# Zokrates/ZoKrates

Hardware: NVIDIA H100
Metric: groth16_constraints_per_sec (higher is better)
Workload: dtype u256-montgomery

## Files before the change

### zokrates_b200/csrc/engine.cuh

```cuda
#pragma once
#include <map>
#include <memory>
#include <vector>
#include <chrono>
#include <cmath>
#include <future>
#include "fp64.cuh"
#include "msm.cuh"
#include "msm_affine.cuh"
#include "ntt.cuh"
#include "ntt_tile.cuh"
#include "solvers.cuh"
#include "rt.cuh"
#include "engine_base.cuh"

#ifndef ZKB_G2_MINB
#define ZKB_G2_MINB 2
#endif

namespace zkb {

struct k_fr_convert; struct k_spmv; struct k_ntt_dif; struct k_ntt_dit; struct k_ntt_scale; struct k_ntt_brev;
struct k_ntt_table; struct k_qap_pointwise; struct k_msm_digits; struct k_msm_scatter; struct k_msm_accum1;
struct k_msm_accum2; struct k_msm_bitsum; struct k_pk_convert; struct k_final_a; struct k_final_b;
struct k_final_c; struct k_final_d; struct k_point_out; struct k_field_op; struct k_setup_scalars; struct k_fixed_base;
struct k_to_affine; struct k_copy; struct k_msm_view; struct k_solver_level; struct k_ba_halve; struct k_ba_round; struct k_msm_table; struct k_ntt_dif_tile; struct k_ntt_dit_tile; struct k_witness_level;

struct StageTimer {
#if !defined(ZKB_EMU)
  struct Ev { const char* name; cudaEvent_t a, b; };
  std::vector<Ev> evs;
  std::vector<size_t> open;
  Stream st;
  explicit StageTimer(Stream s) : st(s) {}
  void begin(const char* name) {
    Ev e{name, nullptr, nullptr};
    ZKB_CUDA(cudaEventCreate(&e.a));
    ZKB_CUDA(cudaEventCreate(&e.b));
    ZKB_CUDA(cudaEventRecord(e.a, st.s));
    open.push_back(evs.size());
    evs.push_back(e);
  }
  void end() {
    size_t i = open.back();
    open.pop_back();
    ZKB_CUDA(cudaEventRecord(evs[i].b, st.s));
  }
  size_t begin_on(Stream s, const char* name) {
    Ev e{name, nullptr, nullptr};
    ZKB_CUDA(cudaEventCreate(&e.a));
    ZKB_CUDA(cudaEventCreate(&e.b));
    ZKB_CUDA(cudaEventRecord(e.a, s.s));
    evs.push_back(e);
    return evs.size() - 1;
  }
  void end_on(Stream s, size_t i) { ZKB_CUDA(cudaEventRecord(evs[i].b, s.s)); }
  void collect(std::vector<std::pair<const char*, double>>& out) {
    out.clear();
    for (auto& e : evs) {
      ZKB_CUDA(cudaEventSynchronize(e.b));
      float ms = 0;
      ZKB_CUDA(cudaEventElapsedTime(&ms, e.a, e.b));
      out.push_back({e.name, (double)ms});
      cudaEventDestroy(e.a);
      cudaEventDestroy(e.b);
    }
    evs.clear();
  }
  ~StageTimer() { for (auto& e : evs) { cudaEventDestroy(e.a); cudaEventDestroy(e.b); } }
#else
  explicit StageTimer(Stream) {}
  void begin(const char*) {}
  void end() {}
  size_t begin_on(Stream, const char*) { return 0; }
  void end_on(Stream, size_t) {}
  void collect(std::vector<std::pair<const char*, double>>& out) { out.clear(); }
#endif
};

#if !defined(ZKB_EMU)
static __global__ void zkb_scan_kernel(const uint32_t* counts, uint32_t* offsets, uint32_t n) {
  __shared__ uint32_t sums[1024];
  const uint32_t tid = threadIdx.x;
  const uint32_t per = (n + 1023u) / 1024u;
  const uint32_t lo = tid * per < n ? tid * per : n;
  const uint32_t hi = lo + per < n ? lo + per : n;
  uint32_t s = 0;
  for (uint32_t i = lo; i < hi; i++) s += counts[i];
  sums[tid] = s;
  __syncthreads();
  for (uint32_t off = 1; off < 1024; off <<= 1) {
    uint32_t v = tid >= off ? sums[tid - off] : 0;
    __syncthreads();
    sums[tid] += v;
    __syncthreads();
  }
  uint32_t base = tid ? sums[tid - 1] : 0;
  for (uint32_t i = lo; i < hi; i++) {
    offsets[i] = base;
    base += counts[i];
  }
  if (tid == 1023) offsets[n] = sums[1023];
}
#endif
#if !defined(ZKB_EMU)
static constexpr int SCAN_BLOCK = 256, SCAN_PER = 8, SCAN_TILE = SCAN_BLOCK * SCAN_PER;
static __global__ void zkb_scan_tile_sums(const uint32_t* in, uint32_t* tile_sums, uint32_t n) {
  __shared__ uint32_t red[SCAN_BLOCK / 32];
  const uint32_t base = blockIdx.x * SCAN_TILE + threadIdx.x * SCAN_PER;
  uint32_t s = 0;
#pragma unroll
  for (int k = 0; k < SCAN_PER; k++) s += (base + k < n) ? in[base + k] : 0;
  for (int off = 16; off; off >>= 1) s += __shfl_down_sync(0xffffffffu, s, off);
  if ((threadIdx.x & 31) == 0) red[threadIdx.x >> 5] = s;
  __syncthreads();
  if (threadIdx.x == 0) {
    uint32_t t = 0;
    for (int k = 0; k < SCAN_BLOCK / 32; k++) t += red[k];
    tile_sums[blockIdx.x] = t;
  }
}
static __global__ void zkb_scan_tile_apply(const uint32_t* in, const uint32_t* tile_offsets, uint32_t* out, uint32_t n,
                                           uint32_t ntiles) {
  __shared__ uint32_t wsum[SCAN_BLOCK / 32];
  const uint32_t base = blockIdx.x * SCAN_TILE + threadIdx.x * SCAN_PER;
  uint32_t v[SCAN_PER], s = 0;
#pragma unroll
  for (int k = 0; k < SCAN_PER; k++) { v[k] = (base + k < n) ? in[base + k] : 0; s += v[k]; }
  uint32_t incl = s;
  const uint32_t lane = threadIdx.x & 31, warp = threadIdx.x >> 5;
  for (int off = 1; off < 32; off <<= 1) { uint32_t y = __shfl_up_sync(0xffffffffu, incl, off); if (lane >= (uint32_t)off) incl += y; }
  if (lane == 31) wsum[warp] = incl;
  __syncthreads();
  uint32_t wbase = 0;
  for (uint32_t k = 0; k < warp; k++) wbase += wsum[k];
  uint32_t run = tile_offsets[blockIdx.x] + wbase + incl - s;
#pragma unroll
  for (int k = 0; k < SCAN_PER; k++) { if (base + k < n) out[base + k] = run; run += v[k]; }
  if (blockIdx.x == ntiles - 1 && threadIdx.x == SCAN_BLOCK - 1) out[n] = tile_offsets[ntiles];
}
#endif
inline void exclusive_scan(Stream st, const uint32_t* counts, uint32_t* offsets, uint32_t n, uint32_t* tile_tmp = nullptr) {
#if !defined(ZKB_EMU)
  if (tile_tmp && n > 4096) {
    const uint32_t ntiles = (n + SCAN_TILE - 1) / SCAN_TILE;
    launch_counter() += 3;
    zkb_scan_tile_sums<<<ntiles, SCAN_BLOCK, 0, st.s>>>(counts, tile_tmp, n);
    zkb_scan_kernel<<<1, 1024, 0, st.s>>>(tile_tmp, tile_tmp + ntiles + 1, ntiles);
    zkb_scan_tile_apply<<<ntiles, SCAN_BLOCK, 0, st.s>>>(counts, tile_tmp + ntiles + 1, offsets, n, ntiles);
    ZKB_CUDA(cudaGetLastError());
    return;
  }
  launch_counter()++;
  zkb_scan_kernel<<<1, 1024, 0, st.s>>>(counts, offsets, n);
  ZKB_CUDA(cudaGetLastError());
#else
  (void)tile_tmp;
  uint32_t base = 0;
  for (uint32_t i = 0; i < n; i++) { offsets[i] = base; base += counts[i]; }
  offsets[n] = base;
#endif
}

static constexpr int VIEW_BLOCK = 256, VIEW_ITERS = 8, VIEW_TILE = VIEW_BLOCK * VIEW_ITERS, VIEW_GROUPS = VIEW_TILE / 32;
#if !defined(ZKB_EMU)
static __global__ void __launch_bounds__(VIEW_BLOCK) zkb_view_count(MsmShape sh, const uint8_t* skip, const uint32_t* sorted0,
                                                                    const uint32_t* offsets0, uint32_t NB, uint32_t* tile_cnt,
                                                                    uint32_t ntiles) {
  __shared__ uint32_t cnt[2];
  if (threadIdx.x < 2) cnt[threadIdx.x] = 0;
  __syncthreads();
// ... 733 lines not shown
    pl.sh.W = (C::FR_BITS + 1 + c - 1) / c;
    pl.sh.B = 1u << (c - 1);
    pl.nbuckets = msm_nbuckets(pl.sh);
    uint64_t total = n * pl.sh.W;
    if (total * nviews >= (1ull << 32)) throw Error(ZKB_E_ARG, "msm too large");
    uint64_t target = (uint64_t)opts.chunk_target;
    uint64_t T = (total + target - 1) / target;
    if (T < 8) T = 8;
    if (T > 64) T = 64;
    T = (T + 1) & ~1ull;
    pl.T1 = (uint32_t)T;
    pl.T2 = 8;
    pl.nt1 = (uint32_t)((total + pl.T1 - 1) / pl.T1);
    const uint32_t NB = pl.nbuckets;
    if (nviews > 3) throw Error(ZKB_E_INTERNAL, "at most two filtered views");
    pl.digits.ensure(total); pl.ranks.ensure(total); pl.sorted.ensure(total * nviews);
    pl.counts.ensure(NB); pl.offsets.ensure((size_t)(NB + 1) * nviews);
    dev_zero(st_, pl.counts.p, (size_t)NB * 4);
    MsmShape sh = pl.sh;
    const uint32_t* sc = (const uint32_t*)scalars;
    uint32_t* dg = pl.digits.p; uint32_t* rk = pl.ranks.p; uint32_t* cn = pl.counts.p; uint32_t* of = pl.offsets.p;
    uint32_t* so = pl.sorted.p;
    launch<k_msm_digits>(st_, n, ZKB_LAMBDA(size_t t) { msm_digits_body(sh, sc, dg, rk, cn, (uint32_t)t); });
    const uint32_t ntiles = (uint32_t)((total + VIEW_TILE - 1) / VIEW_TILE);
    pl.scan_tmp.ensure(2 * ((size_t)(NB > ntiles ? NB : ntiles) / 2048 + 4));
    exclusive_scan(st_, cn, of, NB, pl.scan_tmp.p);
    launch<k_msm_scatter>(st_, total, ZKB_LAMBDA(size_t t) { msm_scatter_body(sh, dg, rk, of, so, t); });
    if (nviews > 1) build_views(pl, skip, total, ntiles);
  }

  void build_views(MsmPlan& pl, const uint8_t* skip, uint64_t total, uint32_t ntiles) {
    const uint32_t NB = pl.nbuckets, nv = pl.nviews - 1;
    const MsmShape sh = pl.sh;
    const uint32_t* of0 = pl.offsets.p;
    const uint32_t* so0 = pl.sorted.p;
    uint32_t* sov = pl.sorted.p + total;
#if !defined(ZKB_EMU)
    const uint32_t ngroups = (uint32_t)((total + 31) / 32);
    pl.view_tile_cnt.ensure((size_t)2 * ntiles); pl.view_tile_off.ensure((size_t)2 * (ntiles + 1));
    pl.view_pre32.ensure((size_t)2 * ngroups); pl.view_mask32.ensure((size_t)2 * ngroups);
    launch_counter() += 2;
    zkb_view_count<<<ntiles, VIEW_BLOCK, 0, st_.s>>>(sh, skip, so0, of0, NB, pl.view_tile_cnt.p, ntiles);
    ZKB_CUDA(cudaGetLastError());
    for (uint32_t v = 0; v < nv; v++)
      exclusive_scan(st_, pl.view_tile_cnt.p + (size_t)v * ntiles, pl.view_tile_off.p + (size_t)v * (ntiles + 1), ntiles, pl.scan_tmp.p);
    zkb_view_apply<<<ntiles, VIEW_BLOCK, 0, st_.s>>>(sh, skip, so0, of0, NB, nv, pl.view_tile_off.p, ntiles, sov, (size_t)total,
                                                     pl.view_pre32.p, pl.view_mask32.p, ngroups);
    ZKB_CUDA(cudaGetLastError());
    for (uint32_t v = 0; v < nv; v++) {
      const uint32_t* pre = pl.view_pre32.p + (size_t)v * ngroups; const uint32_t* msk = pl.view_mask32.p + (size_t)v * ngroups;
      const uint32_t* tot = pl.view_tile_off.p + (size_t)v * (ntiles + 1) + ntiles;
      uint32_t* ofv = pl.offsets.p + (size_t)(v + 1) * (NB + 1);
      launch<k_msm_view>(st_, (size_t)NB + 1, ZKB_LAMBDA(size_t t) { msm_view_offsets_body(NB, of0, pre, msk, tot, ofv, (uint32_t)t); });
    }
#else
    (void)ntiles;
    const uint32_t M = of0[NB];
    for (uint32_t v = 0; v < nv; v++) {
      uint32_t* ofv = pl.offsets.p + (size_t)(v + 1) * (NB + 1);
      uint32_t* out = sov + (size_t)v * total;
      uint32_t kept = 0, b = 0;
      for (uint32_t p = 0; p <= M; p++) {
        while (b <= NB && of0[b] == p) ofv[b++] = kept;
        if (p < M && msm_view_keep(sh, skip, so0[p], v + 1)) out[kept++] = so0[p];
      }
    }
#endif
  }

  MsmWs ws_misc_;
  Stream wm_stream_, plan_stream_;
  bool has_wm_stream_ = false, has_plan_stream_ = false;
  struct StreamScope {
    Stream& ref; Stream saved;
    StreamScope(Stream& r, Stream s) : ref(r), saved(r) { ref = s; }
    ~StreamScope() { ref = saved; }
  };
  Stream tail_stream(MsmWs& ws) {
    if (!ws.has_stream) { ws.tail = stream_create_high_priority(); ws.has_stream = true; }
    return ws.tail;
  }
  ~Engine() override {
    if (prepared_.fut.valid()) prepared_.fut.wait();
    for (auto& sl : slots_) { if (sl.fm.valid()) sl.fm.wait(); sl.destroy(); }
    ws_misc_.destroy();
    if (has_wm_stream_) stream_destroy(wm_stream_);
    if (has_plan_stream_) stream_destroy(plan_stream_);
  }

  DevBuf<uint8_t> ba_pts_[2];
  DevBuf<uint32_t> ba_off_[2], ba_cnt_, ba_scan_tmp_;

  template <class F>
  void msm_accumulate(const MsmPlan& pl, const Affine<F>* pts, MsmWs& ws, StageTimer* tm, const char* accum_name, uint32_t view) {
    typedef XYZZ<F> X;
    if (pl.sh.n == 0) return;
    const uint32_t NB = pl.nbuckets;
    ws.buckets.ensure((size_t)NB * sizeof(X));
    X* buckets = (X*)ws.buckets.p;
    const uint32_t* of = pl.offsets.p + (size_t)view * (NB + 1);
    const uint32_t* so = pl.sorted.p + (size_t)view * pl.sh.n * pl.sh.W;
    uint64_t bound = (uint64_t)pl.sh.n * pl.sh.W;
    uint32_t rounds = 0;
    if (opts.batch_affine > 0 && bound >= ((uint64_t)1 << opts.batch_affine_min_log) && bound < (1ull << 31)) rounds = (uint32_t)opts.batch_affine;
    ws.tail_done.wait(st_);
    if (tm && accum_name) tm->begin(accum_name);
    const Affine<F>* cur_pts = pts;
    for (uint32_t r = 0; r < rounds; r++) {
      const uint64_t out_bound = (bound + NB) / 2 + 1;
      ba_cnt_.ensure(NB); ba_off_[r & 1].ensure((size_t)NB + 1); ba_scan_tmp_.ensure(2 * ((size_t)NB / 2048 + 4));
      ba_pts_[r & 1].ensure(out_bound * sizeof(Affine<F>));
      const uint32_t* off_in = of;
      uint32_t* cnt = ba_cnt_.p; uint32_t* off_out = ba_off_[r & 1].p;
      launch<k_ba_halve>(st_, NB, ZKB_LAMBDA(size_t t) { ba_halve_counts_body(NB, off_in, cnt, (uint32_t)t); });
      exclusive_scan(st_, cnt, off_out, NB, ba_scan_tmp_.p);
      Affine<F>* out = (Affine<F>*)ba_pts_[r & 1].p;
      const uint32_t* srt = so;
      const Affine<F>* pin = cur_pts;
#if !defined(ZKB_EMU)
      {
        constexpr int MINB = sizeof(F) > sizeof(Fq) ? 2 : 3;
        static bool configured = false;
        if (!configured) {
          ZKB_CUDA(cudaFuncSetAttribute(zkb_batch_affine<F, MINB>, cudaFuncAttributeMaxDynamicSharedMemorySize, (int)ba_smem_bytes<F>()));
          configured = true;
        }
        const size_t blocks = (size_t)((out_bound + BA_TILE - 1) / BA_TILE);
        launch_counter()++;
        zkb_batch_affine<F, MINB><<<(unsigned)blocks, BA_BLOCK, ba_smem_bytes<F>(), st_.s>>>(NB, off_in, off_out, srt, pin, out);
        ZKB_CUDA(cudaGetLastError());
      }
#else
      {
        const size_t blocks = (size_t)((out_bound + BA_TILE - 1) / BA_TILE);
        launch_counter()++;
        for (size_t blk = 0; blk < blocks; blk++) ba_block_emulate<F>(NB, off_in, off_out, srt, pin, out, (uint32_t)blk);
      }
#endif
      of = off_out; so = nullptr; cur_pts = out; bound = out_bound;
    }
    uint32_t T1 = pl.T1, nt1 = pl.nt1;
    if (rounds) {
      uint64_t T = (bound + 600000 - 1) / 600000;
      if (T < 8) T = 8;
      if (T > 64) T = 64;
      T1 = (uint32_t)((T + 1) & ~1ull);
      nt1 = (uint32_t)((bound + T1 - 1) / T1);
    }
    ws.nt1 = nt1;
    for (int k = 0; k < 2; k++) { ws.key[k].ensure(2 * (size_t)nt1 + 2); ws.val[k].ensure((2 * (size_t)nt1 + 2) * sizeof(X)); }
    dev_zero(st_, buckets, (size_t)NB * sizeof(X));
    uint32_t* k0 = ws.key[0].p; X* v0 = (X*)ws.val[0].p;
    const Affine<F>* fin_pts = cur_pts;
    if (sizeof(F) > sizeof(Fq)) {
      launch<k_msm_accum1, 128, ZKB_G2_MINB>(st_, nt1, ZKB_LAMBDA(size_t t) { msm_accum1_body<F>(NB, T1, of, so, fin_pts, buckets, k0, v0, nt1, (uint32_t)t); });
    } else {
      launch<k_msm_accum1>(st_, nt1, ZKB_LAMBDA(size_t t) { msm_accum1_body<F>(NB, T1, of, so, fin_pts, buckets, k0, v0, nt1, (uint32_t)t); });
    }
    if (tm && accum_name) tm->end();
    ws.acc_done.record(st_);
  }

  template <class F>
  void msm_tail(const MsmPlan& pl, MsmWs& ws, XYZZ<F>* win_out , StageTimer* tm = nullptr, const char* tail_name = nullptr) {
    typedef XYZZ<F> X;
    if (pl.sh.n == 0) return;
    Stream ts = tail_stream(ws);
    ws.acc_done.wait(ts);
    size_t span = (tm && tail_name) ? tm->begin_on(ts, tail_name) : 0;
    const uint32_t W = pl.sh.pre ? 1 : pl.sh.W, B = pl.sh.B, T2 = pl.T2, nt1 = ws.nt1;
    X* buckets = (X*)ws.buckets.p;
    uint32_t L = 2 * nt1;
    int cur = 0;
    while (true) {
      uint32_t nt = L / T2 + 1;
      const uint32_t* ik = ws.key[cur].p; const X* iv = (const X*)ws.val[cur].p;
      uint32_t* ok = ws.key[cur ^ 1].p; X* ov = (X*)ws.val[cur ^ 1].p;
      uint32_t Lc = L;
      launch<k_msm_accum2>(ts, nt, ZKB_LAMBDA(size_t t) { msm_accum2_body<F>(Lc, T2, ik, iv, buckets, ok, ov, nt, (uint32_t)t); });
      if (nt == 1) break;
      L = 2 * nt;
      cur ^= 1;
    }
    const uint32_t rbits = opts.bitsum_radix == 8 ? 3u : 1u;
    const size_t half = ((size_t)W * B) >> 1;
    if (rbits == 3) {
      const size_t first = (size_t)W * (B >> 3);
      ws.tree[0].ensure((first + 1) * sizeof(X)); ws.tree[1].ensure((first / 8 + 1) * sizeof(X));
      ws.tree[2].ensure((3 * first + 1) * sizeof(X)); ws.tree[3].ensure((3 * first + 1) * sizeof(X));
    } else {
      ws.tree[0].ensure((half + 1) * sizeof(X)); ws.tree[1].ensure((half / 2 + 1) * sizeof(X));
      ws.tree[2].ensure((half + 1) * sizeof(X)); ws.tree[3].ensure((half + 1) * sizeof(X));
    }
    const X* inA = buckets; const X* inP = nullptr;
    uint32_t cnt = B, lvl = 0, nbits = 0;
    const size_t host_nodes = sizeof(F) > sizeof(Fq) ? HOST_TREE_NODES / 8 : HOST_TREE_NODES;
    while (cnt >= (1u << rbits) && (size_t)W * cnt > host_nodes) {
      X* oA = (X*)ws.tree[lvl & 1].p; X* oP = (X*)ws.tree[2 + (lvl & 1)].p;
      const X* iA = inA; const X* iP = inP;
      const uint32_t ci = cnt, np = nbits;
      if (rbits == 3) {
        const size_t threads = (size_t)(4 + np) * W * (cnt >> 3);
        launch<k_msm_bitsum>(ts, threads, ZKB_LAMBDA(size_t t) { msm_bitsum_body<F>(W, ci, np, iA, iP, oA, oP, (uint32_t)t); });
      } else {
        const size_t threads = (size_t)(2 + np) * W * (cnt >> 1);
        launch<k_msm_bitsum, 64>(ts, threads, ZKB_LAMBDA(size_t t) { msm_bitsum2_body<F>(W, ci, np, iA, iP, oA, oP, (uint32_t)t); });
      }
      inA = oA; inP = oP; cnt >>= rbits; lvl++; nbits += rbits;
    }
    ws.tree_cnt = cnt; ws.tree_bits = nbits;
    const size_t nodes = (size_t)W * cnt;
    ws.out_entries = nodes * (1 + (size_t)nbits);
    if (ws.out_entries > MAXW) throw Error(ZKB_E_INTERNAL, "msm result slot overflow");
    d2d(ts, win_out, inA, nodes * sizeof(X));
    if (nbits) d2d(ts, win_out + nodes, inP, nodes * nbits * sizeof(X));
    if (tm && tail_name) tm->end_on(ts, span);
    ws.tail_done.record(ts);
  }

  template <class F>
  void msm_exec(const MsmPlan& pl, const Affine<F>* pts, XYZZ<F>* win_out, MsmWs& ws, StageTimer* tm = nullptr,
                const char* accum_name = nullptr, uint32_t view = 0, const char* tail_name = nullptr) {
    msm_accumulate<F>(pl, pts, ws, tm, accum_name, view);
    msm_tail<F>(pl, ws, win_out, tm, tail_name);
  }

  static constexpr size_t HOST_TREE_NODES = 32;
  template <class HX>
  static HX host_finish(const HX* slot, const MsmPlan& pl, const MsmWs& ws) {
    const uint32_t W = pl.sh.pre ? 1 : pl.sh.W, cnt = ws.tree_cnt, nbits = ws.tree_bits, c = pl.sh.c;
    const size_t nodes = (size_t)W * cnt;
    const HX* A = slot;
    auto window_sum = [&](uint32_t w) {
      HX run = HX::identity(), hi = HX::identity();
      for (uint32_t k = cnt; k-- > 0;) {
        run = HX::add(run, A[(size_t)w * cnt + k]);
        if (k > 0) hi = HX::add(hi, run);
      }
      for (uint32_t bit = nbits; bit-- > 0;) {
        const HX* P = slot + nodes * (1 + (size_t)bit) + (size_t)w * cnt;
        HX sb = HX::identity();
        for (uint32_t k = 0; k < cnt; k++) sb = HX::add(sb, P[k]);
        hi = HX::add(HX::dbl(hi), sb);
      }
      return HX::add(hi, run);
    };
    std::vector<HX> S(W);
    if (W >= 8) {
      auto part = [&](uint32_t q) { for (uint32_t w = q; w < W; w += 4) S[w] = window_sum(w); };
      std::future<void> f1 = std::async(std::launch::async, part, 1u), f2 = std::async(std::launch::async, part, 2u),
                        f3 = std::async(std::launch::async, part, 3u);
      part(0);
      f1.get(); f2.get(); f3.get();
    } else {
      for (uint32_t w = 0; w < W; w++) S[w] = window_sum(w);
    }
    HX acc = HX::identity();
    for (uint32_t w = W; w-- > 0;) {
      if (w + 1 < W) for (uint32_t d = 0; d < c; d++) acc = HX::dbl(acc);
      acc = HX::add(acc, S[w]);
    }
    return acc;
  }

  struct Pk {
    uint64_t ni = 0, m = 0, hl = 0, ll = 0;
    uint32_t rank = 0, world = 1;
    uint64_t lo = 0, hi = 0, hlo = 0, hhi = 0;
    DevBuf<G1A> a, b1, l, h;
    DevBuf<G2A> b2;
    DevBuf<G1A> fixed1;
    DevBuf<G2A> fixed2;
    uint32_t pre_cz = 0, pre_ch = 0;
    int z_status = 0, h_status = 0;
    size_t table_bytes = 0;
    DevBuf<uint8_t> skip;
    HG1A h_fixed1[5];
    HG2A h_fixed2[3];
    uint64_t fp[2] = {0, 0};
  };
  std::map<uint64_t, std::shared_ptr<Pk>> pks_;
  std::shared_ptr<Pk> idle_pk_;
  static void fingerprint(const uint8_t* data, size_t len, uint64_t salt, uint64_t out[2]) {
    uint64_t h[4] = {0x9E3779B97F4A7C15ull ^ salt, 0xC2B2AE3D27D4EB4Full + len, 0x165667B19E3779F9ull, 0x27D4EB2F165667C5ull ^ (salt << 17)};
    const uint64_t k1 = 0xff51afd7ed558ccdull, k2 = 0xc4ceb9fe1a85ec53ull;
    size_t i = 0;
    for (; i + 32 <= len; i += 32) {
      uint64_t w[4];
      memcpy(w, data + i, 32);
      for (int l = 0; l < 4; l++) { uint64_t x = (h[l] ^ w[l]) * k1; h[l] = ((x << 29) | (x >> 35)) + k2; }
    }
    uint8_t tail[32] = {0};
    memcpy(tail, data + i, len - i);
    uint64_t w[4];
    memcpy(w, tail, 32);
    for (int l = 0; l < 4; l++) { uint64_t x = (h[l] ^ w[l]) * k2; h[l] = ((x << 31) | (x >> 33)) * k1; }
    auto mix = [&](uint64_t x) { x ^= x >> 33; x *= k1; x ^= x >> 29; x *= k2; x ^= x >> 32; return x; };
    out[0] = mix(h[0] + mix(h[1])) ^ mix(h[2] ^ (h[3] << 1));
    out[1] = mix(h[2] + mix(h[3] ^ k1)) + mix(h[0] ^ (h[1] >> 3));
  }
  static void fingerprint_par(const uint8_t* data, size_t len, uint64_t salt, uint64_t out[2]) {
    constexpr int PARTS = 8;
    if (len < ((size_t)8 << 20)) { fingerprint(data, len, salt, out); return; }
    uint64_t part[PARTS][2];
    std::vector<std::future<void>> fs;
    const size_t step = ((len / PARTS) + 31) & ~(size_t)31;
    for (int k = 0; k < PARTS; k++) {
      const size_t lo = std::min(len, step * k), hi = k == PARTS - 1 ? len : std::min(len, step * (k + 1));
// ... 701 lines not shown
```

### zokrates_b200/csrc/msm.cuh

```cuda
#pragma once
#include "ec.cuh"

namespace zkb {

static constexpr uint32_t MSM_NONE = 0xFFFFFFFFu;
static constexpr uint32_t MSM_NEG = 0x80000000u;

#if defined(__CUDA_ARCH__)
__device__ __forceinline__ uint32_t zkb_atomic_add(uint32_t* p, uint32_t v) { return atomicAdd(p, v); }
#else
inline uint32_t zkb_atomic_add(uint32_t* p, uint32_t v) { uint32_t o = *p; *p = o + v; return o; }
#endif

struct MsmShape {
  uint32_t n;
  uint32_t c;
  uint32_t W;
  uint32_t B;
  uint32_t pre;
};
ZKB_HD uint32_t msm_nbuckets(const MsmShape& sh) { return sh.pre ? sh.B : sh.W * sh.B; }

ZKB_HD uint32_t scalar_bits(const uint32_t* s, uint32_t lo, uint32_t cnt) {
  uint32_t limb = lo >> 5, sh = lo & 31;
  uint64_t v = limb < 8 ? s[limb] : 0;
  if (limb + 1 < 8) v |= (uint64_t)s[limb + 1] << 32;
  return (uint32_t)(v >> sh) & ((1u << cnt) - 1u);
}

ZKB_HDN inline void msm_digits_body(MsmShape sh, const uint32_t* scalars , uint32_t* digits, uint32_t* ranks,
                                    uint32_t* counts , uint32_t i) {
  if (i >= sh.n) return;
  uint32_t s[8];
#pragma unroll
  for (int k = 0; k < 8; k++) s[k] = scalars[(size_t)i * 8 + k];
  uint32_t carry = 0;
  const uint32_t full = 1u << sh.c, half = sh.B;
  for (uint32_t w = 0; w < sh.W; w++) {
    uint32_t d = scalar_bits(s, w * sh.c, sh.c) + carry;
    uint32_t code;
    if (d == 0) {
      code = MSM_NONE;
      carry = 0;
    } else if (d > half) {
      code = (full - d - 1) | MSM_NEG;
      carry = 1;
      if (full - d == 0) {
        code = MSM_NONE;
      }
    } else {
      code = d - 1;
      carry = 0;
    }
    digits[(size_t)w * sh.n + i] = code;
    if (code != MSM_NONE) {
      const uint32_t key = (sh.pre ? 0u : w * sh.B) + (code & ~MSM_NEG);
      ranks[(size_t)w * sh.n + i] = zkb_atomic_add(&counts[key], 1);
    }
  }
}

ZKB_HDN inline void msm_scatter_body(MsmShape sh, const uint32_t* digits, const uint32_t* ranks, const uint32_t* offsets,
                                     uint32_t* sorted, size_t t) {
  const size_t total = (size_t)sh.n * sh.W;
  if (t >= total) return;
  uint32_t code = digits[t];
  if (code == MSM_NONE) return;
  uint32_t w = (uint32_t)(t / sh.n), i = (uint32_t)(t % sh.n);
  uint32_t key = (sh.pre ? 0u : w * sh.B) + (code & ~MSM_NEG);
  const uint32_t val = (sh.pre ? w * sh.n + i : i) | (code & MSM_NEG);
  sorted[offsets[key] + ranks[t]] = val;
}

ZKB_HD uint32_t msm_view_keep(const MsmShape& sh, const uint8_t* skip, uint32_t entry, uint32_t v) {
  const uint32_t idx = entry & ~MSM_NEG;
  const uint32_t i = sh.pre ? idx % sh.n : idx;
  return !((skip[i] >> (v - 1)) & 1u);
}
ZKB_HDN inline void msm_view_offsets_body(uint32_t NB, const uint32_t* offsets0, const uint32_t* pre32, const uint32_t* mask32,
                                          const uint32_t* total_v, uint32_t* offsets_v, uint32_t b) {
  if (b > NB) return;
  const uint32_t M = offsets0[NB], p = offsets0[b];
  if (p >= M) { offsets_v[b] = *total_v; return; }
  const uint32_t g = p >> 5, lane = p & 31u;
  const uint32_t below = mask32[g] & ((1u << lane) - 1u);
#if defined(__CUDA_ARCH__)
  offsets_v[b] = pre32[g] + __popc(below);
#else
  offsets_v[b] = pre32[g] + (uint32_t)__builtin_popcount(below);
#endif
}

template <class F>
ZKB_HDN inline void msm_accum1_body(uint32_t nbuckets, uint32_t T, const uint32_t* offsets, const uint32_t* sorted,
                                    const Affine<F>* points, XYZZ<F>* buckets, uint32_t* pkey, XYZZ<F>* pval,
                                    uint32_t nthreads, uint32_t t) {
  if (t >= nthreads) return;
  const uint32_t M = offsets[nbuckets];
  uint32_t k0 = MSM_NONE, k1 = MSM_NONE;
  uint64_t start64 = (uint64_t)t * T;
  if (start64 < M) {
    uint32_t pos = (uint32_t)start64;
    uint32_t end = (M - pos > T) ? pos + T : M;
    uint32_t lo = 0, hi = nbuckets;
    while (hi - lo > 1) {
      uint32_t mid = (lo + hi) >> 1;
      if (offsets[mid] <= pos) lo = mid; else hi = mid;
    }
    uint32_t b = lo;
    const uint32_t cstart = pos;
    while (offsets[b + 1] <= pos) b++;
    uint32_t bstart = offsets[b], bend = offsets[b + 1];
    XYZZ<F> acc = XYZZ<F>::identity();
    constexpr bool PREFETCH_POINT = sizeof(Affine<F>) <= 64;
    uint32_t e = sorted ? sorted[pos] : pos;
    Affine<F> q;
    if (PREFETCH_POINT) q = points[e & ~MSM_NEG];
    for (uint32_t p = pos; p < end; p++) {
      uint32_t e_next = 0;
      Affine<F> q_next;
      if (p + 1 < end) {
        e_next = sorted ? sorted[p + 1] : p + 1;
        if (PREFETCH_POINT) q_next = points[e_next & ~MSM_NEG];
      }
      if (p == bend) {
        if (bstart >= cstart) buckets[b] = acc;
        else { k0 = b; pval[2 * (size_t)t] = acc; }
        b++;
        while (offsets[b + 1] <= p) b++;
        bstart = p;
        bend = offsets[b + 1];
        acc = XYZZ<F>::identity();
      }
      if (!PREFETCH_POINT) q = points[e & ~MSM_NEG];
      if (e & MSM_NEG) q.y = F::neg(q.y);
      acc = XYZZ<F>::madd(acc, q);
      e = e_next;
      if (PREFETCH_POINT) q = q_next;
    }
    if (bstart >= cstart && bend <= end) buckets[b] = acc;
    else if (bstart < cstart) { k0 = b; pval[2 * (size_t)t] = acc; }
    else { k1 = b; pval[2 * (size_t)t + 1] = acc; }
  }
  pkey[2 * (size_t)t] = k0;
  pkey[2 * (size_t)t + 1] = k1;
}

template <class F>
ZKB_HDN inline void msm_accum2_body(uint32_t L, uint32_t T, const uint32_t* key, const XYZZ<F>* val, XYZZ<F>* buckets,
                                    uint32_t* okey, XYZZ<F>* oval, uint32_t nthreads, uint32_t t) {
  if (t >= nthreads) return;
  uint64_t s64 = (uint64_t)t * T;
  uint32_t s = s64 == 0 ? 0 : (uint32_t)(s64 - 1);
  uint64_t e64 = s64 + T - 1;
  uint32_t e = e64 < L ? (uint32_t)e64 : L;
  uint32_t k0 = MSM_NONE, k1 = MSM_NONE;
  uint32_t left = MSM_NONE;
  if (s >= 1) {
    left = key[s - 1];
    if (left == MSM_NONE && s >= 2) left = key[s - 2];
  }
  uint32_t right = MSM_NONE;
  if (e < L) {
    right = key[e];
    if (right == MSM_NONE && e + 1 < L) right = key[e + 1];
  }
  uint32_t cur = MSM_NONE;
  XYZZ<F> acc = XYZZ<F>::identity();
  bool first = true;
  for (uint32_t p = s; p <= e; p++) {
    uint32_t k = (p < e) ? key[p] : MSM_NONE - 1;
    if (p < e && k == MSM_NONE) continue;
    if (k != cur) {
      if (cur != MSM_NONE) {
        bool last = (p == e);
        bool open_left = first && left == cur;
        bool open_right = last && right == cur;
        if (!open_left && !open_right) {
          buckets[cur] = acc;
        } else if (open_left) {
          k0 = cur;
          oval[2 * (size_t)t] = acc;
        } else {
          k1 = cur;
          oval[2 * (size_t)t + 1] = acc;
        }
        first = false;
      }
      cur = k;
      acc = XYZZ<F>::identity();
    }
    if (p < e) acc = XYZZ<F>::add(acc, val[p]);
  }
  okey[2 * (size_t)t] = k0;
  okey[2 * (size_t)t + 1] = k1;
}

template <class F, int MAXW>
ZKB_HDN inline void msm_table_body(const Affine<F>* pts, Affine<F>* table, uint32_t n, uint32_t c, uint32_t W, uint32_t i) {
  if (i >= n) return;
  Affine<F> p = pts[i];
  table[i] = p;
  if (p.is_inf()) {
    for (uint32_t w = 1; w < W; w++) table[(size_t)w * n + i] = Affine<F>::inf();
    return;
  }
  XYZZ<F> cur = XYZZ<F>::from_affine(p);
  XYZZ<F> mult[MAXW];
  F pref[MAXW];
  F run = F::one();
  for (uint32_t w = 1; w < W; w++) {
    for (uint32_t d = 0; d < c; d++) cur = XYZZ<F>::dbl_ni(cur);
    mult[w] = cur;
    pref[w] = run;
    run = F::mul_ni(run, F::mul_ni(cur.zz, cur.zzz));
  }
  F inv = F::inv(run);
  for (uint32_t w = W; w-- > 1;) {
    F dinv = F::mul_ni(inv, pref[w]);
    inv = F::mul_ni(inv, F::mul_ni(mult[w].zz, mult[w].zzz));
    F zzi = F::mul_ni(dinv, mult[w].zzz), zzzi = F::mul_ni(dinv, mult[w].zz);
    table[(size_t)w * n + i] = Affine<F>{F::mul_ni(mult[w].x, zzi), F::mul_ni(mult[w].y, zzzi)};
  }
}

template <class F>
ZKB_HDN inline void msm_bitsum_body(uint32_t W, uint32_t cnt_in, uint32_t npend, const XYZZ<F>* inA, const XYZZ<F>* inP,
                                    XYZZ<F>* outA, XYZZ<F>* outP, uint32_t t) {
  const uint32_t cnt_out = cnt_in >> 3;
  const uint32_t per_role = W * cnt_out;
  const uint32_t role = t / per_role, node = t % per_role;
  if (role >= 4 + npend) return;
  const uint32_t w = node / cnt_out, k = node % cnt_out;
  const XYZZ<F>* src = (role < 4 ? inA : inP + (size_t)(role - 4) * W * cnt_in) + (size_t)w * cnt_in + ((size_t)k << 3);
  uint32_t mask = 0xFFu;
  if (role == 1) mask = 0xAAu; else if (role == 2) mask = 0xCCu; else if (role == 3) mask = 0xF0u;
  XYZZ<F> sum = XYZZ<F>::identity();
#pragma unroll 1
  for (uint32_t i = 0; i < 8; i++)
    if ((mask >> i) & 1u) sum = XYZZ<F>::add(sum, src[i]);
  XYZZ<F>* dst;
  if (role == 0) dst = outA;
  else if (role < 4) dst = outP + (size_t)(npend + role - 1) * per_role;
  else dst = outP + (size_t)(role - 4) * per_role;
  dst[node] = sum;
}

template <class F>
ZKB_HDN inline void msm_bitsum2_body(uint32_t W, uint32_t cnt_in, uint32_t npend, const XYZZ<F>* inA, const XYZZ<F>* inP,
                                     XYZZ<F>* outA, XYZZ<F>* outP, uint32_t t) {
  const uint32_t cnt_out = cnt_in >> 1;
  const uint32_t per_role = W * cnt_out;
  const uint32_t role = t / per_role, node = t % per_role;
  if (role >= 2 + npend) return;
  const uint32_t w = node / cnt_out, k = node % cnt_out;
  const bool from_a = role == 0 || role == 1 + npend;
  const XYZZ<F>* src = (from_a ? inA : inP + (size_t)(role - 1) * W * cnt_in) + (size_t)w * cnt_in + ((size_t)k << 1);
  if (role == 0) outA[node] = XYZZ<F>::add(src[0], src[1]);
  else if (role == 1 + npend) outP[(size_t)npend * per_role + node] = src[1];
  else outP[(size_t)(role - 1) * per_role + node] = XYZZ<F>::add(src[0], src[1]);
}

}
```

### zokrates_b200/csrc/msm_affine.cuh

```cuda
#pragma once
#include <vector>
#include "msm.cuh"

namespace zkb {

static constexpr uint32_t BA_M = 8;
static constexpr uint32_t BA_BLOCK = 128;
static constexpr uint32_t BA_TILE = BA_M * BA_BLOCK;

ZKB_HDN inline void ba_halve_counts_body(uint32_t NB, const uint32_t* off_in, uint32_t* cnt_out, uint32_t b) {
  if (b >= NB) return;
  const uint32_t L = off_in[b + 1] - off_in[b];
  cnt_out[b] = (L + 1) >> 1;
}

ZKB_HD uint32_t ba_find_bucket(const uint32_t* off_out, uint32_t NB, uint32_t j) {
  uint32_t lo = 0, hi = NB;
  while (hi - lo > 1) {
    const uint32_t mid = (lo + hi) >> 1;
    if (off_out[mid] <= j) lo = mid; else hi = mid;
  }
  while (off_out[lo + 1] <= j) lo++;
  return lo;
}

enum BaMode : uint32_t { BA_ADD = 0, BA_DBL = 1, BA_COPY1 = 2, BA_COPY2 = 3, BA_INF = 4 };

template <class F>
ZKB_HD Affine<F> ba_load(const uint32_t* sorted, const Affine<F>* pts, uint32_t pos) {
  if (!sorted) return pts[pos];
  const uint32_t e = sorted[pos];
  Affine<F> p = pts[e & ~MSM_NEG];
  if (e & MSM_NEG) p.y = F::neg(p.y);
  return p;
}

template <class F>
ZKB_HD uint32_t ba_mode(const Affine<F>& p1, const Affine<F>& p2, bool has2, F& den) {
  den = F::one();
  if (!has2 || p2.is_inf()) return BA_COPY1;
  if (p1.is_inf()) return BA_COPY2;
  F dx = F::sub(p2.x, p1.x);
  if (!dx.is_zero()) { den = dx; return BA_ADD; }
  if (p1.y == p2.y && !p1.y.is_zero()) { den = F::dbl(p1.y); return BA_DBL; }
  return BA_INF;
}

template <class F>
ZKB_HD Affine<F> ba_finish(uint32_t mode, const Affine<F>& p1, const Affine<F>& p2, const F& dinv) {
  if (mode == BA_COPY1) return p1;
  if (mode == BA_COPY2) return p2;
  if (mode == BA_INF) return Affine<F>::inf();
  F num;
  if (mode == BA_DBL) { F xx = F::sqr(p1.x); num = F::add(F::dbl(xx), xx); }
  else num = F::sub(p2.y, p1.y);
  const F lam = F::mul(num, dinv);
  const F x3 = F::sub(F::sub(F::sqr(lam), p1.x), mode == BA_DBL ? p1.x : p2.x);
  const F y3 = F::sub(F::mul(lam, F::sub(p1.x, x3)), p1.y);
  return Affine<F>{x3, y3};
}

template <class F>
ZKB_HDN inline void ba_round_ref_body(uint32_t NB, const uint32_t* off_in, const uint32_t* off_out, const uint32_t* sorted,
                                      const Affine<F>* pts_in, Affine<F>* pts_out, uint32_t j) {
  if (j >= off_out[NB]) return;
  const uint32_t b = ba_find_bucket(off_out, NB, j);
  const uint32_t pin = off_in[b] + 2 * (j - off_out[b]);
  const bool has2 = pin + 1 < off_in[b + 1];
  const Affine<F> p1 = ba_load<F>(sorted, pts_in, pin);
  Affine<F> p2 = p1;
  if (has2) p2 = ba_load<F>(sorted, pts_in, pin + 1);
  F den;
  const uint32_t mode = ba_mode<F>(p1, p2, has2, den);
  pts_out[j] = ba_finish<F>(mode, p1, p2, mode <= BA_DBL ? F::inv(den) : den);
}

#if !defined(ZKB_EMU)
template <class F>
struct BaVec {
  static constexpr int Q = sizeof(F) / 16;
  static_assert(sizeof(F) % 16 == 0, "16-byte planes");
  uint4* base;
  uint32_t count;
  __device__ __forceinline__ void st(uint32_t i, const F& v) const {
    const uint4* s = (const uint4*)&v;
#pragma unroll
    for (int q = 0; q < Q; q++) base[(size_t)q * count + i] = s[q];
  }
  __device__ __forceinline__ F ld(uint32_t i) const {
    F v;
    uint4* d = (uint4*)&v;
#pragma unroll
    for (int q = 0; q < Q; q++) d[q] = base[(size_t)q * count + i];
    return v;
  }
};
#else
template <class F>
struct BaVec {
  F* base;
  uint32_t count;
  void st(uint32_t i, const F& v) const { base[i] = v; }
  F ld(uint32_t i) const { return base[i]; }
};
#endif

template <class F>
struct BaShared {
  BaVec<F> pref;
  BaVec<F> node;
  BaVec<F> ninv;
};
template <class F>
struct BaThread {
  uint32_t pin[BA_M];
  F run;
};

template <class F>
ZKB_HD void ba_forward(BaThread<F>& th, const BaShared<F>& sh, uint32_t NB, const uint32_t* off_in, const uint32_t* off_out,
                       const uint32_t* sorted, const Affine<F>* pts_in, uint32_t blk, uint32_t tid) {
  const uint32_t M = off_out[NB];
  const uint32_t j0 = (blk * BA_BLOCK + tid) * BA_M;
  F run = F::one();
  uint32_t b = 0, ob = 0, ob1 = 0, ib = 0, ib1 = 0;
  if (j0 < M) { b = ba_find_bucket(off_out, NB, j0); ob = off_out[b]; ob1 = off_out[b + 1]; ib = off_in[b]; ib1 = off_in[b + 1]; }
#pragma unroll
  for (uint32_t k = 0; k < BA_M; k++) {
    const uint32_t j = j0 + k;
    sh.pref.st(k * BA_BLOCK + tid, run);
    if (j >= M) { th.pin[k] = 0xFFFFFFFFu; continue; }
    while (ob1 <= j) { b++; ob = ob1; ob1 = off_out[b + 1]; ib = ib1; ib1 = off_in[b + 1]; }
    const uint32_t p = ib + 2 * (j - ob);
    const bool has2 = p + 1 < ib1;
    th.pin[k] = p | (has2 ? 0x80000000u : 0u);
    const Affine<F> p1 = ba_load<F>(sorted, pts_in, p);
    Affine<F> p2 = p1;
    if (has2) p2 = ba_load<F>(sorted, pts_in, p + 1);
    F den;
    const uint32_t mode = ba_mode<F>(p1, p2, has2, den);
    if (mode <= BA_DBL) run = F::mul(run, den);
  }
  th.run = run;
  sh.node.st(BA_BLOCK + tid, run);
}
template <class F>
ZKB_HD void ba_tree_up(const BaShared<F>& sh, uint32_t s, uint32_t tid) {
  if (tid >= s) return;
  const uint32_t i = s + tid;
  sh.node.st(i, F::mul(sh.node.ld(2 * i), sh.node.ld(2 * i + 1)));
}
template <class F>
ZKB_HD void ba_tree_root(const BaShared<F>& sh, uint32_t tid) {
  if (tid == 0) sh.ninv.st(1, F::inv(sh.node.ld(1)));
}
template <class F>
ZKB_HD void ba_tree_down(const BaShared<F>& sh, uint32_t s, uint32_t tid) {
  if (tid >= s) return;
  const uint32_t i = s + tid;
  const F pi = sh.ninv.ld(i);
  sh.ninv.st(2 * i, F::mul(pi, sh.node.ld(2 * i + 1)));
  sh.ninv.st(2 * i + 1, F::mul(pi, sh.node.ld(2 * i)));
}
template <class F>
ZKB_HD void ba_backward(const BaThread<F>& th, const BaShared<F>& sh, const uint32_t* sorted, const Affine<F>* pts_in, Affine<F>* pts_out,
                        uint32_t blk, uint32_t tid) {
  const uint32_t j0 = (blk * BA_BLOCK + tid) * BA_M;
  F inv = sh.ninv.ld(BA_BLOCK + tid);
#pragma unroll
  for (uint32_t kk = 0; kk < BA_M; kk++) {
    const uint32_t k = BA_M - 1 - kk;
    if (th.pin[k] == 0xFFFFFFFFu) continue;
    const uint32_t p = th.pin[k] & 0x7FFFFFFFu;
    const bool has2 = (th.pin[k] >> 31) != 0;
    const Affine<F> p1 = ba_load<F>(sorted, pts_in, p);
    Affine<F> p2 = p1;
    if (has2) p2 = ba_load<F>(sorted, pts_in, p + 1);
    F den;
    const uint32_t mode = ba_mode<F>(p1, p2, has2, den);
    F dinv = den;
    if (mode <= BA_DBL) {
      dinv = F::mul(inv, sh.pref.ld(k * BA_BLOCK + tid));
      inv = F::mul(inv, den);
    }
    pts_out[j0 + k] = ba_finish<F>(mode, p1, p2, dinv);
  }
}

template <class F>
constexpr size_t ba_smem_bytes() { return (size_t)(BA_TILE + 2 * 2 * BA_BLOCK) * sizeof(F); }

#if !defined(ZKB_EMU)
template <class F, int MINB>
__global__ void __launch_bounds__(BA_BLOCK, MINB) zkb_batch_affine(uint32_t NB, const uint32_t* __restrict__ off_in,
                                                                    const uint32_t* __restrict__ off_out, const uint32_t* __restrict__ sorted,
                                                                    const Affine<F>* __restrict__ pts_in, Affine<F>* __restrict__ pts_out) {
  extern __shared__ uint4 ba_smem[];
  constexpr int Q = BaVec<F>::Q;
  BaShared<F> sh;
  sh.pref = BaVec<F>{ba_smem, BA_TILE};
  sh.node = BaVec<F>{ba_smem + (size_t)Q * BA_TILE, 2 * BA_BLOCK};
  sh.ninv = BaVec<F>{ba_smem + (size_t)Q * (BA_TILE + 2 * BA_BLOCK), 2 * BA_BLOCK};
  if ((uint64_t)blockIdx.x * BA_TILE >= off_out[NB]) return;
  const uint32_t tid = threadIdx.x;
  BaThread<F> th;
  ba_forward<F>(th, sh, NB, off_in, off_out, sorted, pts_in, blockIdx.x, tid);
  __syncthreads();
  for (uint32_t s = BA_BLOCK >> 1; s >= 1; s >>= 1) { ba_tree_up<F>(sh, s, tid); __syncthreads(); }
  ba_tree_root<F>(sh, tid);
  __syncthreads();
  for (uint32_t s = 1; s < BA_BLOCK; s <<= 1) { ba_tree_down<F>(sh, s, tid); __syncthreads(); }
  ba_backward<F>(th, sh, sorted, pts_in, pts_out, blockIdx.x, tid);
}
#else
template <class F>
inline void ba_block_emulate(uint32_t NB, const uint32_t* off_in, const uint32_t* off_out, const uint32_t* sorted, const Affine<F>* pts_in,
                             Affine<F>* pts_out, uint32_t blk) {
  if ((uint64_t)blk * BA_TILE >= off_out[NB]) return;
  std::vector<F> pref(BA_TILE), node(2 * BA_BLOCK), ninv(2 * BA_BLOCK);
  std::vector<BaThread<F>> th(BA_BLOCK);
  BaShared<F> sh{BaVec<F>{pref.data(), BA_TILE}, BaVec<F>{node.data(), 2 * BA_BLOCK}, BaVec<F>{ninv.data(), 2 * BA_BLOCK}};
  for (uint32_t t = 0; t < BA_BLOCK; t++) ba_forward<F>(th[t], sh, NB, off_in, off_out, sorted, pts_in, blk, t);
  for (uint32_t s = BA_BLOCK >> 1; s >= 1; s >>= 1) for (uint32_t t = 0; t < BA_BLOCK; t++) ba_tree_up<F>(sh, s, t);
  for (uint32_t t = 0; t < BA_BLOCK; t++) ba_tree_root<F>(sh, t);
  for (uint32_t s = 1; s < BA_BLOCK; s <<= 1) for (uint32_t t = 0; t < BA_BLOCK; t++) ba_tree_down<F>(sh, s, t);
  for (uint32_t t = 0; t < BA_BLOCK; t++) ba_backward<F>(th[t], sh, sorted, pts_in, pts_out, blk, t);
}
#endif

}
```

Measured before the change: 52.04 million.

## Keep G2 bucket accumulator in shared memory with cp.async double-buffered point loads

```diff
diff --git a/zokrates_b200/csrc/engine.cuh b/zokrates_b200/csrc/engine.cuh
--- a/zokrates_b200/csrc/engine.cuh
+++ b/zokrates_b200/csrc/engine.cuh
@@ -13,10 +13,6 @@
 #include "solvers.cuh"
 #include "rt.cuh"
 #include "engine_base.cuh"
-
-#ifndef ZKB_G2_MINB
-#define ZKB_G2_MINB 2
-#endif
 
 namespace zkb {
 
@@ -1056,8 +1052,29 @@
     dev_zero(st_, buckets, (size_t)NB * sizeof(X));
     uint32_t* k0 = ws.key[0].p; X* v0 = (X*)ws.val[0].p;
     const Affine<F>* fin_pts = cur_pts;
-    if (sizeof(F) > sizeof(Fq)) {
-      launch<k_msm_accum1, 128, ZKB_G2_MINB>(st_, nt1, ZKB_LAMBDA(size_t t) { msm_accum1_body<F>(NB, T1, of, so, fin_pts, buckets, k0, v0, nt1, (uint32_t)t); });
+    if constexpr (sizeof(F) > sizeof(Fq)) {
+      constexpr uint32_t BLOCK = 128;
+      constexpr size_t smem = msm_accum1_shared_bytes<F>(BLOCK);
+      const size_t blocks = (nt1 + BLOCK - 1) / BLOCK;
+      if (blocks) launch_counter()++;
+#if !defined(ZKB_EMU)
+      constexpr int MINB = sizeof(Fq) == 32 ? 3 : 2;
+      static bool configured = false;
+      if (!configured) {
+        ZKB_CUDA(cudaFuncSetAttribute(zkb_msm_accum1_shared<F, BLOCK, MINB>, cudaFuncAttributeMaxDynamicSharedMemorySize, (int)smem));
+        configured = true;
+      }
+      if (blocks) {
+        zkb_msm_accum1_shared<F, BLOCK, MINB><<<(unsigned)blocks, BLOCK, smem, st_.s>>>(NB, T1, of, so, fin_pts, buckets, k0, v0, nt1);
+        ZKB_CUDA(cudaGetLastError());
+      }
+#else
+      std::vector<F> sbuf(smem / sizeof(F));
+      const BaVec<F> sm{sbuf.data(), 8 * BLOCK};
+      for (size_t blk = 0; blk < blocks; blk++)
+        for (uint32_t tid = 0; tid < BLOCK; tid++)
+          msm_accum1_shared_body<F>(NB, T1, of, so, fin_pts, buckets, k0, v0, nt1, (uint32_t)blk * BLOCK + tid, sm, tid, BLOCK);
+#endif
     } else {
       launch<k_msm_accum1>(st_, nt1, ZKB_LAMBDA(size_t t) { msm_accum1_body<F>(NB, T1, of, so, fin_pts, buckets, k0, v0, nt1, (uint32_t)t); });
     }
diff --git a/zokrates_b200/csrc/msm.cuh b/zokrates_b200/csrc/msm.cuh
--- a/zokrates_b200/csrc/msm.cuh
+++ b/zokrates_b200/csrc/msm.cuh
@@ -145,6 +145,170 @@
   pkey[2 * (size_t)t] = k0;
   pkey[2 * (size_t)t + 1] = k1;
 }
+
+#if !defined(ZKB_EMU)
+template <class F>
+struct BaVec {
+  static constexpr int Q = sizeof(F) / 16;
+  static_assert(sizeof(F) % 16 == 0, "16-byte planes");
+  uint4* base;
+  uint32_t count;
+  __device__ __forceinline__ void st(uint32_t i, const F& v) const {
+    const uint4* s = (const uint4*)&v;
+#pragma unroll
+    for (int q = 0; q < Q; q++) base[(size_t)q * count + i] = s[q];
+  }
+  __device__ __forceinline__ F ld(uint32_t i) const {
+    F v;
+    uint4* d = (uint4*)&v;
+#pragma unroll
+    for (int q = 0; q < Q; q++) d[q] = base[(size_t)q * count + i];
+    return v;
+  }
+  __device__ __forceinline__ void ld_async(uint32_t i, const F* src) const {
+#pragma unroll
+    for (int q = 0; q < Q; q++) {
+      const uint32_t s = (uint32_t)__cvta_generic_to_shared(base + (size_t)q * count + i);
+      asm volatile("cp.async.cg.shared.global [%0], [%1], 16;" ::"r"(s), "l"((const uint4*)src + q) : "memory");
+    }
+  }
+};
+ZKB_HD void cp_async_commit() {
+#if defined(__CUDA_ARCH__)
+  asm volatile("cp.async.commit_group;" ::: "memory");
+#endif
+}
+template <int N>
+ZKB_HD void cp_async_wait() {
+#if defined(__CUDA_ARCH__)
+  asm volatile("cp.async.wait_group %0;" ::"n"(N) : "memory");
+#endif
+}
+#else
+template <class F>
+struct BaVec {
+  F* base;
+  uint32_t count;
+  void st(uint32_t i, const F& v) const { base[i] = v; }
+  F ld(uint32_t i) const { return base[i]; }
+  void ld_async(uint32_t i, const F* src) const { base[i] = *src; }
+};
+inline void cp_async_commit() {}
+template <int N>
+inline void cp_async_wait() {}
+#endif
+
+template <class F>
+ZKB_HD void msm_madd_shared(const BaVec<F>& sm, uint32_t a , uint32_t q , uint32_t stride) {
+  const uint32_t ax = a, ay = a + stride, azz = a + 2 * stride, azzz = a + 3 * stride, qx = q, qy = q + stride;
+  if (Affine<F>{sm.ld(qx), sm.ld(qy)}.is_inf()) return;
+  if (sm.ld(azz).is_zero()) {
+    sm.st(ax, sm.ld(qx)); sm.st(ay, sm.ld(qy)); sm.st(azz, F::one()); sm.st(azzz, F::one());
+    return;
+  }
+  const F U2 = F::mul(sm.ld(qx), sm.ld(azz));
+  const F S2 = F::mul(sm.ld(qy), sm.ld(azzz));
+  const F Pd = F::sub(U2, sm.ld(ax));
+  const F Rd = F::sub(S2, sm.ld(ay));
+  if (Pd.is_zero()) {
+    const XYZZ<F> r = Rd.is_zero() ? XYZZ<F>::mdbl_ni(Affine<F>{sm.ld(qx), sm.ld(qy)}) : XYZZ<F>::identity();
+    sm.st(ax, r.x); sm.st(ay, r.y); sm.st(azz, r.zz); sm.st(azzz, r.zzz);
+    return;
+  }
+  const F PP = F::sqr(Pd);
+  sm.st(azz, F::mul(sm.ld(azz), PP));
+  const F PPP = F::mul(Pd, PP);
+  const F Q = F::mul(sm.ld(ax), PP);
+  const F X3 = F::sub(F::sub(F::sqr(Rd), PPP), F::dbl(Q));
+  sm.st(ax, X3);
+  sm.st(ay, F::mul_sub(Rd, F::sub(Q, X3), sm.ld(ay), PPP));
+  sm.st(azzz, F::mul(sm.ld(azzz), PPP));
+}
+
+template <class F>
+ZKB_HD void msm_xyzz_st(const BaVec<F>& sm, uint32_t a, uint32_t stride, const XYZZ<F>& v) {
+  sm.st(a, v.x); sm.st(a + stride, v.y); sm.st(a + 2 * stride, v.zz); sm.st(a + 3 * stride, v.zzz);
+}
+template <class F>
+ZKB_HD XYZZ<F> msm_xyzz_ld(const BaVec<F>& sm, uint32_t a, uint32_t stride) {
+  return XYZZ<F>{sm.ld(a), sm.ld(a + stride), sm.ld(a + 2 * stride), sm.ld(a + 3 * stride)};
+}
+
+template <class F>
+ZKB_HDN inline void msm_accum1_shared_body(uint32_t nbuckets, uint32_t T, const uint32_t* offsets, const uint32_t* sorted,
+                                           const Affine<F>* points, XYZZ<F>* buckets, uint32_t* pkey, XYZZ<F>* pval,
+                                           uint32_t nthreads, uint32_t t, const BaVec<F>& sm, uint32_t tid, uint32_t block) {
+  if (t >= nthreads) return;
+  const uint32_t M = offsets[nbuckets];
+  uint32_t k0 = MSM_NONE, k1 = MSM_NONE;
+  uint64_t start64 = (uint64_t)t * T;
+  if (start64 < M) {
+    uint32_t pos = (uint32_t)start64;
+    uint32_t end = (M - pos > T) ? pos + T : M;
+    uint32_t lo = 0, hi = nbuckets;
+    while (hi - lo > 1) {
+      uint32_t mid = (lo + hi) >> 1;
+      if (offsets[mid] <= pos) lo = mid; else hi = mid;
+    }
+    uint32_t b = lo;
+    const uint32_t cstart = pos;
+    while (offsets[b + 1] <= pos) b++;
+    uint32_t bstart = offsets[b], bend = offsets[b + 1];
+    const uint32_t acc = tid, pt = 4 * block + tid;
+    msm_xyzz_st(sm, acc, block, XYZZ<F>::identity());
+    uint32_t e = sorted ? sorted[pos] : pos;
+    uint32_t e_next = pos + 1 < end ? (sorted ? sorted[pos + 1] : pos + 1) : 0;
+    sm.ld_async(pt, &points[e & ~MSM_NEG].x);
+    sm.ld_async(pt + block, &points[e & ~MSM_NEG].y);
+    cp_async_commit();
+    for (uint32_t p = pos; p < end; p++) {
+      const uint32_t cur = pt + ((p - pos) & 1) * 2 * block, nxt = pt + ((p - pos + 1) & 1) * 2 * block;
+      uint32_t e_next2 = 0;
+      if (p + 1 < end) {
+        sm.ld_async(nxt, &points[e_next & ~MSM_NEG].x);
+        sm.ld_async(nxt + block, &points[e_next & ~MSM_NEG].y);
+        if (p + 2 < end) e_next2 = sorted ? sorted[p + 2] : p + 2;
+      }
+      cp_async_commit();
+      cp_async_wait<1>();
+      if (p == bend) {
+        const XYZZ<F> v = msm_xyzz_ld(sm, acc, block);
+        if (bstart >= cstart) buckets[b] = v;
+        else { k0 = b; pval[2 * (size_t)t] = v; }
+        b++;
+        while (offsets[b + 1] <= p) b++;
+        bstart = p;
+        bend = offsets[b + 1];
+        msm_xyzz_st(sm, acc, block, XYZZ<F>::identity());
+      }
+      if (e & MSM_NEG) sm.st(cur + block, F::neg(sm.ld(cur + block)));
+      msm_madd_shared(sm, acc, cur, block);
+      e = e_next;
+      e_next = e_next2;
+    }
+    const XYZZ<F> v = msm_xyzz_ld(sm, acc, block);
+    if (bstart >= cstart && bend <= end) buckets[b] = v;
+    else if (bstart < cstart) { k0 = b; pval[2 * (size_t)t] = v; }
+    else { k1 = b; pval[2 * (size_t)t + 1] = v; }
+  }
+  pkey[2 * (size_t)t] = k0;
+  pkey[2 * (size_t)t + 1] = k1;
+}
+
+template <class F>
+constexpr size_t msm_accum1_shared_bytes(uint32_t block) { return (size_t)8 * block * sizeof(F); }
+
+#if !defined(ZKB_EMU)
+template <class F, int BLOCK, int MINB>
+__global__ void __launch_bounds__(BLOCK, MINB) zkb_msm_accum1_shared(uint32_t nbuckets, uint32_t T, const uint32_t* __restrict__ offsets,
+                                                                     const uint32_t* __restrict__ sorted, const Affine<F>* __restrict__ points,
+                                                                     XYZZ<F>* buckets, uint32_t* pkey, XYZZ<F>* pval, uint32_t nthreads) {
+  extern __shared__ uint4 acc_smem[];
+  const BaVec<F> sm{acc_smem, 8 * BLOCK};
+  msm_accum1_shared_body<F>(nbuckets, T, offsets, sorted, points, buckets, pkey, pval, nthreads, blockIdx.x * BLOCK + threadIdx.x, sm,
+                            threadIdx.x, BLOCK);
+}
+#endif
 
 template <class F>
 ZKB_HDN inline void msm_accum2_body(uint32_t L, uint32_t T, const uint32_t* key, const XYZZ<F>* val, XYZZ<F>* buckets,
diff --git a/zokrates_b200/csrc/msm_affine.cuh b/zokrates_b200/csrc/msm_affine.cuh
--- a/zokrates_b200/csrc/msm_affine.cuh
+++ b/zokrates_b200/csrc/msm_affine.cuh
@@ -74,36 +74,6 @@
   const uint32_t mode = ba_mode<F>(p1, p2, has2, den);
   pts_out[j] = ba_finish<F>(mode, p1, p2, mode <= BA_DBL ? F::inv(den) : den);
 }
-
-#if !defined(ZKB_EMU)
-template <class F>
-struct BaVec {
-  static constexpr int Q = sizeof(F) / 16;
-  static_assert(sizeof(F) % 16 == 0, "16-byte planes");
-  uint4* base;
-  uint32_t count;
-  __device__ __forceinline__ void st(uint32_t i, const F& v) const {
-    const uint4* s = (const uint4*)&v;
-#pragma unroll
-    for (int q = 0; q < Q; q++) base[(size_t)q * count + i] = s[q];
-  }
-  __device__ __forceinline__ F ld(uint32_t i) const {
-    F v;
-    uint4* d = (uint4*)&v;
-#pragma unroll
-    for (int q = 0; q < Q; q++) d[q] = base[(size_t)q * count + i];
-    return v;
-  }
-};
-#else
-template <class F>
-struct BaVec {
-  F* base;
-  uint32_t count;
-  void st(uint32_t i, const F& v) const { base[i] = v; }
-  F ld(uint32_t i) const { return base[i]; }
-};
-#endif
 
 template <class F>
 struct BaShared {
```

New measurement: 52.94 million, median of 6. 1.02x the previous value.
